# shiinamiyuki/akari_render

Hardware: AMD Instinct MI355X
Metric: Msamples/s (whole node), 1080p path tracer, C2 (higher is better)
Workload: dtype f32

## Files before the change

### akari_render_amd/csrc/device/disect.h

```cpp
#pragma once
#include "drng.h"
#include "dscene.h"
#include "../kernels.h"

namespace akr {

template <bool V>
struct BoolTag {
    static constexpr bool value = V;
};

struct Hit {
    float t, u, v;
    uint32_t gid;
};

struct PlaneHit {
    float t, px, py, pz;
};
AKR_HD PlaneHit tri_plane(vec3 o, vec3 d, float4 r2) {
    float dz = __builtin_fmaf(r2.x, d.x, __builtin_fmaf(r2.y, d.y, r2.z * d.z));
    float oz = __builtin_fmaf(r2.x, o.x, __builtin_fmaf(r2.y, o.y, __builtin_fmaf(r2.z, o.z, r2.w)));
    PlaneHit h;
    h.t = div_f(-oz, dz);
    h.px = __builtin_fmaf(h.t, d.x, o.x);
    h.py = __builtin_fmaf(h.t, d.y, o.y);
    h.pz = __builtin_fmaf(h.t, d.z, o.z);
    return h;
}
AKR_HD void tri_uv(const PlaneHit& h, float4 r0, float4 r1, float& u, float& v) {
    u = __builtin_fmaf(r0.x, h.px, __builtin_fmaf(r0.y, h.py, __builtin_fmaf(r0.z, h.pz, r0.w)));
    v = __builtin_fmaf(r1.x, h.px, __builtin_fmaf(r1.y, h.py, __builtin_fmaf(r1.z, h.pz, r1.w)));
}
AKR_HD bool tri_test(vec3 o, vec3 d, float4 r0, float4 r1, float4 r2, float tmin, float tmax, float& t_out, float& u_out,
                     float& v_out) {
    PlaneHit h = tri_plane(o, d, r2);
    float u, v;
    tri_uv(h, r0, r1, u, v);
    t_out = h.t;
    u_out = u;
    v_out = v;
    return (h.t >= tmin) & (h.t <= tmax) & (u >= 0.0f) & (v >= 0.0f) & (u + v <= 1.0f);
}

AKR_D float textured_alpha(const DScene& sc, const float4* r, uint32_t material, float u, float v) {
    float w = 1.0f - u - v;
    vec2 uv = mk2((r[0].w * w + r[2].w * u) + r[4].w * v, (r[1].w * w + r[3].w * u) + r[5].w * v);
    return material_alpha_at(sc.tex, sc.materials[material], material, uv);
}
template <bool TEX>
AKR_D bool alpha_test(const DScene& sc, uint32_t gid, float u, float v) {
    const float4* r = sc.shade + (size_t)gid * SHADE_ROWS;
    float4 q6 = r[6];
    const DMaterial& m = sc.materials[f2u(q6.y)];
    float alpha = (m.kind == MAT_PRINCIPLED || m.kind == MAT_DIFFUSE) ? m.base_alpha : 1.0f;
    if (TEX) {
        if (m.flags & MF_ALPHA_TEXTURED)
            alpha = textured_alpha(sc, r, f2u(q6.y), u, v);
    }
    if (alpha >= 1.0f) return true;
    uint32_t inst = f2u(q6.z);
    uint32_t prim = gid - sc.inst_tri_offset[inst];
    float h = (float)xxhash32_4(inst, prim, f2u(u), f2u(v)) * 2.3283064365386963e-10f;
    return alpha > h;
}

AKR_D float next_up(float x) {
    uint32_t b = f2u(x);
    return x > 0.0f ? u2f(b + 1u) : (x < 0.0f ? u2f(b - 1u) : u2f(1u));
}
AKR_D float hit_margin(float t, float u, float v, float tmax) {
    return __builtin_fminf(__builtin_fminf(__builtin_fminf(u, v), 1.0f - (u + v)), __builtin_fminf(t, tmax - t));
}

template <bool ANY_HIT, bool TEX = false>
AKR_D bool trace_exhaustive(const DScene& sc, vec3 o, vec3 d, float tmin, float tmax, uint32_t ex0, uint32_t ex1, Hit& hit) {
    float best_t = next_up(tmax);
    uint32_t best = kInvalid;
    float best_u = 0.0f, best_v = 0.0f;
    const uint32_t n = sc.n_tris;
    typedef const float __attribute__((address_space(4))) * ConstF;
    ConstF recs = (ConstF)(uintptr_t)sc.woop;
    auto load_rec = [&](uint32_t k, float4& a, float4& b, float4& c) {
        ConstF r = recs + 12 * (size_t)k;
        a = make_float4(r[0], r[1], r[2], r[3]);
        b = make_float4(r[4], r[5], r[6], r[7]);
        c = make_float4(r[8], r[9], r[10], r[11]);
    };
    float4 n0, n1, n2;
    load_rec(0, n0, n1, n2);
    PlaneHit ph{0.0f, 0.0f, 0.0f, 0.0f};
    for (uint32_t k = 0; k < n; k++) {
        const float4 r0 = n0, r1 = n1, r2 = n2;
        load_rec(k + 1, n0, n1, n2);
        if (!((sc.plane_share_mask >> k) & 1ull)) ph = tri_plane(o, d, r2);
        float u, v;
        const float t = ph.t;
        tri_uv(ph, r0, r1, u, v);
        float m = __builtin_fminf(hit_margin(t, u, v, tmax), t - tmin);
        m = (k == ex0) ? -1.0f : m;
        m = (k == ex1) ? -1.0f : m;
        if (sc.has_alpha) {
            if (m >= 0.0f && !alpha_test<TEX>(sc, k, u, v)) m = -1.0f;
        }
        if (ANY_HIT) {
            if (m >= 0.0f) best = k;
            if (__builtin_amdgcn_ballot_w64(best == kInvalid) == 0) break;
        } else {
            const float tc = (m >= 0.0f) ? t : __builtin_inff();
            const bool better = tc < best_t;
            best_t = better ? tc : best_t;
            best_u = better ? u : best_u;
            best_v = better ? v : best_v;
            best = better ? k : best;
        }
    }
    hit.t = best != kInvalid ? best_t : tmax;
    hit.u = best_u;
    hit.v = best_v;
    hit.gid = best;
    return best != kInvalid;
}

typedef float v2f __attribute__((ext_vector_type(2)));
typedef float v4f __attribute__((ext_vector_type(4)));
AKR_D float min_raw(float a, float b) {
    float r;
    asm("v_min_f32 %0, %1, %2" : "=v"(r) : "v"(a), "v"(b));
    return r;
}
AKR_D float max_raw(float a, float b) {
    float r;
    asm("v_max_f32 %0, %1, %2" : "=v"(r) : "v"(a), "v"(b));
    return r;
}
AKR_D float min_abs_raw(float a, float b) {
    float r;
    asm("v_min_f32 %0, %1, |%2|" : "=v"(r) : "v"(a), "v"(b));
    return r;
}
AKR_D float max3_abs_raw(float a, float b, float c) {
    float r;
    asm("v_max3_f32 %0, |%1|, |%2|, |%3|" : "=v"(r) : "v"(a), "v"(b), "v"(c));
    return r;
}
AKR_D PlaneHit tri_plane_unscaled(vec3 o, vec3 d, float4 r2, float& lo) {
    float dz = __builtin_fmaf(r2.x, d.x, __builtin_fmaf(r2.y, d.y, r2.z * d.z));
    float oz = __builtin_fmaf(r2.x, o.x, __builtin_fmaf(r2.y, o.y, __builtin_fmaf(r2.z, o.z, r2.w)));
    lo = min_abs_raw(lo, oz);
    PlaneHit h;
    h.t = div_f_unscaled(-oz, dz);
    h.px = __builtin_fmaf(h.t, d.x, o.x);
    h.py = __builtin_fmaf(h.t, d.y, o.y);
    h.pz = __builtin_fmaf(h.t, d.z, o.z);
    return h;
}

template <bool DIV>
struct WalkOpt {
    static constexpr bool unscaled_div = DIV;
};
template <int V>
struct IntTag {
    static constexpr int value = V;
};

template <bool TEX = false, class OPT = WalkOpt<true>>
AKR_D void trace_pair_exhaustive(const DScene& sc, vec3 o, vec3 d, float tmax, uint32_t ex0, vec3 so, vec3 sd, float stmax,
                                 uint32_t sex0, uint32_t sex1, Hit& hit, bool& found, bool& occluded, const float4* lds_recs, uint32_t* took_ieee_walk = nullptr) {
    constexpr bool UNSCALED = OPT::unscaled_div && !AKR_RX;
    float best_t = next_up(tmax);
    uint32_t best = kInvalid;
    float best_u = 0.0f, best_v = 0.0f;
    float occ_margin = -1.0f;
    const uint32_t n = sc.n_tris;
    const v4f* lrec = (const v4f*)lds_recs;
    const bool has_alpha = __builtin_amdgcn_readfirstlane((int)sc.has_alpha) != 0;
    float T = 0.0f, srange = 0.0f;
    v2f hx2 = {0.0f, 0.0f}, hy2 = {0.0f, 0.0f}, hz2 = {0.0f, 0.0f};
    float lo = __builtin_inff(), slo = __builtin_inff();
    auto record = [&](auto alpha_tag, auto div_tag, uint32_t k, const v4f& q0, const v4f& q1, const v4f& q2) {
        constexpr int ALPHA = decltype(alpha_tag)::value;
        constexpr bool FAST = decltype(div_tag)::value;
        if (!((sc.plane_share_mask >> k) & 1ull)) {
            const float4 r2 = make_float4(q2.x, q2.y, q2.z, q2.w);
            const PlaneHit a = FAST ? tri_plane_unscaled(o, d, r2, lo) : tri_plane(o, d, r2), b = FAST ? tri_plane_unscaled(so, sd, r2, slo) : tri_plane(so, sd, r2);
            T = a.t;
            srange = min_raw(b.t, stmax - b.t);
            hx2 = (v2f){a.px, b.px}; hy2 = (v2f){a.py, b.py}; hz2 = (v2f){a.pz, b.pz};
        }
        float u, v, su, sv;
        tri_uv(PlaneHit{T, hx2.x, hy2.x, hz2.x}, make_float4(q0.x, q0.y, q0.z, q0.w), make_float4(q1.x, q1.y, q1.z, q1.w), u, v);
        tri_uv(PlaneHit{0.0f, hx2.y, hy2.y, hz2.y}, make_float4(q0.x, q0.y, q0.z, q0.w), make_float4(q1.x, q1.y, q1.z, q1.w), su, sv);
        const v2f u2 = {u, su}, v2 = {v, sv};
        const v2f s2 = {1.0f - (u2.x + v2.x), 1.0f - (u2.y + v2.y)};
        const float range = ALPHA == 0 ? T : min_raw(T, tmax - T);
        float m = min_raw(min_raw(min_raw(u2.x, v2.x), s2.x), range);
        float sm = min_raw(min_raw(min_raw(u2.y, v2.y), s2.y), srange);
        m = (k == ex0) ? -1.0f : m;
        sm = (k == sex0) ? -1.0f : sm;
        sm = (k == sex1) ? -1.0f : sm;
        if (ALPHA == 1 || (ALPHA == 2 && has_alpha)) {
            const uint32_t ka = __builtin_amdgcn_readfirstlane(k);
            if (m >= 0.0f && !alpha_test<TEX>(sc, ka, u2.x, v2.x)) m = -1.0f;
            if (sm >= 0.0f && !alpha_test<TEX>(sc, ka, u2.y, v2.y)) sm = -1.0f;
        }
        const bool better = (m >= 0.0f) & (T < best_t);
        best_t = better ? T : best_t;
        best = better ? k : best;
        occ_margin = max_raw(occ_margin, sm);
    };
    auto walk = [&](auto alpha_tag) {
        const BoolTag<UNSCALED> div_tag{};
        v4f a0 = lrec[0], a1 = lrec[1], a2 = lrec[2], b0, b1, b2;
        uint32_t k = 0;
        for (; k + 1 < n; k += 2) {
            b0 = lrec[3 * (k + 1)]; b1 = lrec[3 * (k + 1) + 1]; b2 = lrec[3 * (k + 1) + 2];
            record(alpha_tag, div_tag, k, a0, a1, a2);
            a0 = lrec[3 * (k + 2)]; a1 = lrec[3 * (k + 2) + 1]; a2 = lrec[3 * (k + 2) + 2];
            record(alpha_tag, div_tag, k + 1, b0, b1, b2);
        }
        if (k < n) record(alpha_tag, div_tag, k, a0, a1, a2);
    };
    auto walk_ieee = [&] {
        best_t = next_up(tmax); best = kInvalid; occ_margin = -1.0f;
#pragma clang loop unroll(disable)
        for (uint32_t k = 0; k < n; k++) {
            record(IntTag<2>{}, BoolTag<false>{}, k, lrec[3 * k], lrec[3 * k + 1], lrec[3 * k + 2]);
        }
    };
    if (UNSCALED) {
        const float ob = lds_recs[3u * (n + 1u) + 2u].w;
        const bool pre_bad = ((tmax >= 0.0f) & !((max3_abs_raw(o.x, o.y, o.z) <= ob) & (max3_abs_raw(d.x, d.y, d.z) <= 2.0f) & (tmax <= 1e20f))) |
                             ((stmax >= 0.0f) & !((max3_abs_raw(so.x, so.y, so.z) <= ob) & (max3_abs_raw(sd.x, sd.y, sd.z) <= 2.0f) & (stmax <= 1e20f)));
        bool redo = __builtin_amdgcn_ballot_w64(pre_bad) != 0;
        if (!redo) {
            if (has_alpha) walk(IntTag<1>{});
            else walk(IntTag<0>{});
            const bool bad = ((tmax >= 0.0f) & (lo < 0x1p-47f)) | ((stmax >= 0.0f) & (slo < 0x1p-47f));
            redo = __builtin_amdgcn_ballot_w64(bad) != 0;
        }
        if (redo) walk_ieee();
        if (took_ieee_walk) *took_ieee_walk = redo ? 1u : 0u;
    } else {
        if (has_alpha) walk(IntTag<1>{});
        else walk(IntTag<0>{});
        if (took_ieee_walk) *took_ieee_walk = 0u;
    }
    if (best != kInvalid) {
        const v4f q0 = lrec[3 * best], q1 = lrec[3 * best + 1];
        const float px = __builtin_fmaf(best_t, d.x, o.x), py = __builtin_fmaf(best_t, d.y, o.y), pz = __builtin_fmaf(best_t, d.z, o.z);
        best_u = __builtin_fmaf(q0.x, px, __builtin_fmaf(q0.y, py, __builtin_fmaf(q0.z, pz, q0.w)));
        best_v = __builtin_fmaf(q1.x, px, __builtin_fmaf(q1.y, py, __builtin_fmaf(q1.z, pz, q1.w)));
    }
    found = best != kInvalid;
    hit.t = found ? best_t : tmax;
    hit.u = best_u;
    hit.v = best_v;
    hit.gid = best;
    occluded = occ_margin >= 0.0f;
}

constexpr uint32_t kBvhDone = 0xfffffffeu;

struct TraceCounters {
    uint32_t nodes, tris, overflow;
};

AKR_D float safe_inv(float d) {
    float a = abs_f(d) < 1e-20f ? __builtin_copysignf(1e-20f, d) : d;
    return __builtin_amdgcn_rcpf(a);
}
AKR_D uint32_t byte_of(uint32_t w, int i) { return (w >> (8 * i)) & 0xffu; }

struct Trav {
    vec3 o, d, inv, noi;
    float tmin, tmax, best_t, best_u, best_v;
    uint32_t ex0, ex1, best;
    uint32_t G, T, tbase, sp, octinv4;
    bool active;
};
AKR_D void trav_begin(Trav& s, vec3 o, vec3 d, float tmin, float tmax, uint32_t ex0, uint32_t ex1) {
    s.o = o; s.d = d;
    s.inv = mk3(safe_inv(d.x), safe_inv(d.y), safe_inv(d.z));
    s.noi = mk3(-o.x * s.inv.x, -o.y * s.inv.y, -o.z * s.inv.z);
    s.tmin = tmin; s.tmax = tmax;
    s.best_t = tmax; s.best_u = 0.0f; s.best_v = 0.0f; s.best = kInvalid;
    s.ex0 = ex0; s.ex1 = ex1;
    const uint32_t oi = (s.inv.x >= 0.0f ? 1u : 0u) | (s.inv.y >= 0.0f ? 2u : 0u) | (s.inv.z >= 0.0f ? 4u : 0u);
    s.octinv4 = oi * 0x01010101u;
    s.G = 1u << (24u + oi);
    s.T = 0; s.tbase = 0; s.sp = 0;
    s.active = tmax >= tmin;
}

AKR_D uint32_t node_pop(Trav& s, uint32_t* __restrict__ stack, uint32_t depth, TraceCounters& cnt) {
    const uint32_t j = 31u - (uint32_t)__builtin_clz(s.G);
    s.G &= ~(1u << j);
    if ((s.G >> 24) != 0) {
        if (s.sp < depth) {
            stack[s.sp * 256u] = s.G;
            s.sp++;
        } else {
            cnt.overflow = 1;
        }
    }
    const uint32_t slot = (j - 24u) ^ (s.octinv4 & 7u);
    return (s.G & 0xffffffu) + slot;
}
AKR_D void hit_commit(Trav& s, bool any_hit, uint32_t gid, float t, float u, float v) {
    if (any_hit) {
        s.best = gid;
        s.T = 0; s.G = 0; s.sp = 0;
    } else {
        const bool better = (s.best == kInvalid) | (t < s.best_t) | ((t == s.best_t) & (gid < s.best));
        if (better) { s.best_t = t; s.best_u = u; s.best_v = v; s.best = gid; }
    }
}
template <bool TEX>
AKR_D void hit_accept(const DScene& sc, Trav& s, bool any_hit, uint32_t gid, float t, float u, float v) {
    bool h = (gid != s.ex0) & (gid != s.ex1);
    if (h && sc.has_alpha) h = alpha_test<TEX>(sc, gid, u, v);
    if (h) hit_commit(s, any_hit, gid, t, u, v);
}

template <int MODE, bool TEX, bool TILE = false>
AKR_D void trav_step_staged(const DScene& sc, Trav& s, uint32_t* __restrict__ stack, TraceCounters& cnt, bool any_rt = false, const uint4* tile = nullptr) {
    const bool any_hit = MODE == 2 ? any_rt : (MODE == 1);
    if (s.T == 0) {
        if ((s.G >> 24) == 0) {
            s.sp--;
            s.G = stack[s.sp * 256u];
        }
        const uint32_t idx = node_pop(s, stack, sc.bvh_stack_depth, cnt);
        const uint4* p = sc.bvh_nodes + (size_t)idx * (kBvhNodeWords / 4);
        uint4 w0, w1, w2, w3;
        if (TILE && idx < sc.bvh_tile_nodes) {
            typedef const volatile uint32_t __attribute__((address_space(3))) * LdsW;
            typedef uint32_t u32x4 __attribute__((ext_vector_type(4)));
            typedef const volatile u32x4 __attribute__((address_space(3))) * LdsU4;
            LdsU4 pt = (LdsU4)((LdsW)(const uint32_t*)tile + idx * kBvhNodeWords);
            const u32x4 t0 = pt[0], t1 = pt[1], t2 = pt[2], t3 = pt[3];
            w0 = make_uint4(t0.x, t0.y, t0.z, t0.w); w1 = make_uint4(t1.x, t1.y, t1.z, t1.w); w2 = make_uint4(t2.x, t2.y, t2.z, t2.w);
            w3 = make_uint4(t3.x, t3.y, t3.z, t3.w);
        } else {
            w0 = p[0]; w1 = p[1]; w2 = p[2]; w3 = p[3];
        }
        cnt.nodes++;
        const float limit = s.best_t;
        const float bx = u2f((w0.w & 0xffu) << 23) * s.inv.x, by = u2f(((w0.w >> 8) & 0xffu) << 23) * s.inv.y, bz = u2f(((w0.w >> 16) & 0xffu) << 23) * s.inv.z;
        const float ax = __builtin_fmaf(u2f(w0.x), s.inv.x, s.noi.x), ay = __builtin_fmaf(u2f(w0.y), s.inv.y, s.noi.y), az = __builtin_fmaf(u2f(w0.z), s.inv.z, s.noi.z);
        const bool nx = s.inv.x < 0.0f, ny = s.inv.y < 0.0f, nz = s.inv.z < 0.0f;
        const uint32_t xb = nx ? ((w3.y >> 16) | (w3.y << 16)) : w3.y, yb = ny ? ((w3.z >> 16) | (w3.z << 16)) : w3.z, zb = nz ? ((w3.w >> 16) | (w3.w << 16)) : w3.w;
        const uint32_t qnx[2] = {nx ? w2.z : w1.w, xb}, qfx[2] = {nx ? w1.w : w2.z, xb >> 16};
        const uint32_t qny[2] = {ny ? w2.w : w2.x, yb}, qfy[2] = {ny ? w2.x : w2.w, yb >> 16};
        const uint32_t qnz[2] = {nz ? w3.x : w2.y, zb}, qfz[2] = {nz ? w2.y : w3.x, zb >> 16};
        uint32_t hitmask = 0;
#pragma unroll
        for (int h = 0; h < 2; h++) {
            const uint32_t meta4 = h ? (w1.x >> 16) : w1.y;
            const uint32_t is_inner4 = (meta4 & (meta4 << 1)) & 0x10101010u;
            const uint32_t inner_mask4 = (is_inner4 >> 4) * 0xffu;
            const uint32_t bit_index4 = (meta4 ^ (s.octinv4 & inner_mask4)) & 0x1f1f1f1fu;
            const uint32_t child_bits4 = (meta4 >> 5) & 0x07070707u;
#pragma unroll
            for (int i = 0; i < (h ? 2 : 4); i++) {
                const float tnx = __builtin_fmaf((float)byte_of(qnx[h], i), bx, ax), tfx = __builtin_fmaf((float)byte_of(qfx[h], i), bx, ax);
                const float tny = __builtin_fmaf((float)byte_of(qny[h], i), by, ay), tfy = __builtin_fmaf((float)byte_of(qfy[h], i), by, ay);
                const float tnz = __builtin_fmaf((float)byte_of(qnz[h], i), bz, az), tfz = __builtin_fmaf((float)byte_of(qfz[h], i), bz, az);
                const float tn = __builtin_fmaxf(__builtin_fmaxf(tnx, tny), __builtin_fmaxf(tnz, s.tmin));
                const float tf = __builtin_fminf(__builtin_fminf(tfx, tfy), __builtin_fminf(tfz, limit));
                if (tn <= tf) hitmask |= byte_of(child_bits4, i) << byte_of(bit_index4, i);
            }
        }
        s.G = ((w0.w >> 24) | ((w1.x & 0xffffu) << 8)) | (hitmask & 0xff000000u);
        s.T = hitmask & 0x00ffffffu;
        s.tbase = w1.z;
    }
    if (s.T != 0) {
        const uint32_t b = (uint32_t)__builtin_ctz(s.T);
        s.T &= s.T - 1u;
        const uint4* p = (const uint4*)sc.woop + (size_t)(s.tbase + b) * (kBvhTriWords / 4);
        const uint4 w0 = p[0], w1 = p[1], w2 = p[2], w3 = p[3];
        cnt.tris++;
        float t, u, v;
        bool h = tri_test(s.o, s.d, make_float4(u2f(w0.x), u2f(w0.y), u2f(w0.z), u2f(w0.w)), make_float4(u2f(w1.x), u2f(w1.y), u2f(w1.z), u2f(w1.w)),
                          make_float4(u2f(w2.x), u2f(w2.y), u2f(w2.z), u2f(w2.w)), s.tmin, s.tmax, t, u, v);
        if (h) hit_accept<TEX>(sc, s, any_hit, w3.x, t, u, v);
    }
    s.active = (s.T != 0) | ((s.G >> 24) != 0) | (s.sp != 0);
}
template <int MODE, bool TEX, bool TILE = false>
AKR_D void trav_step(const DScene& sc, Trav& s, uint32_t* __restrict__ stack, TraceCounters& cnt, bool any_rt = false, const uint4* tile = nullptr) {
    if constexpr (TEX) {
        trav_step_staged<MODE, TEX, TILE>(sc, s, stack, cnt, any_rt, tile);
        return;
    }
    const bool any_hit = MODE == 2 ? any_rt : (MODE == 1);
    const bool do_tri = s.T != 0;
    const uint4* p;
    bool in_tile = false;
    uint32_t tile_idx = 0;
    if (do_tri) {
        const uint32_t b = (uint32_t)__builtin_ctz(s.T);
        s.T &= s.T - 1u;
        p = (const uint4*)sc.woop + (size_t)(s.tbase + b) * (kBvhTriWords / 4);
    } else {
        if ((s.G >> 24) == 0) {
            s.sp--;
            s.G = stack[s.sp * 256u];
        }
        const uint32_t idx = node_pop(s, stack, sc.bvh_stack_depth, cnt);
        p = sc.bvh_nodes + (size_t)idx * (kBvhNodeWords / 4);
        if (TILE && idx < sc.bvh_tile_nodes) {
            in_tile = true;
            tile_idx = idx;
        }
    }
    uint4 w0, w1, w2, w3;
    if (TILE && in_tile) {
        typedef const volatile uint32_t __attribute__((address_space(3))) * LdsW;
        typedef uint32_t u32x4 __attribute__((ext_vector_type(4)));
        typedef const volatile u32x4 __attribute__((address_space(3))) * LdsU4;
        LdsU4 pt = (LdsU4)((LdsW)(const uint32_t*)tile + tile_idx * kBvhNodeWords);
        const u32x4 t0 = pt[0], t1 = pt[1], t2 = pt[2], t3 = pt[3];
        w0 = make_uint4(t0.x, t0.y, t0.z, t0.w); w1 = make_uint4(t1.x, t1.y, t1.z, t1.w); w2 = make_uint4(t2.x, t2.y, t2.z, t2.w);
        w3 = make_uint4(t3.x, t3.y, t3.z, t3.w);
    } else {
        w0 = p[0]; w1 = p[1]; w2 = p[2]; w3 = p[3];
    }
    asm volatile("" : "+v"(w0.x), "+v"(w0.y), "+v"(w0.z), "+v"(w0.w), "+v"(w1.x), "+v"(w1.y), "+v"(w1.z), "+v"(w1.w), "+v"(w2.x), "+v"(w2.y),
                      "+v"(w2.z), "+v"(w2.w), "+v"(w3.x), "+v"(w3.y), "+v"(w3.z), "+v"(w3.w));
    if (do_tri) {
        cnt.tris++;
        float t, u, v;
        bool h = tri_test(s.o, s.d, make_float4(u2f(w0.x), u2f(w0.y), u2f(w0.z), u2f(w0.w)), make_float4(u2f(w1.x), u2f(w1.y), u2f(w1.z), u2f(w1.w)),
                          make_float4(u2f(w2.x), u2f(w2.y), u2f(w2.z), u2f(w2.w)), s.tmin, s.tmax, t, u, v);
        if (h) {
            const uint32_t gid = w3.x;
            h = (gid != s.ex0) & (gid != s.ex1);
            if (h && sc.has_alpha) h = alpha_test<TEX>(sc, gid, u, v);
            if (h) {
                if (any_hit) {
                    s.best = gid;
                    s.T = 0; s.G = 0; s.sp = 0;
                } else {
                    const bool better = (s.best == kInvalid) | (t < s.best_t) | ((t == s.best_t) & (gid < s.best));
                    if (better) { s.best_t = t; s.best_u = u; s.best_v = v; s.best = gid; }
                }
            }
        }
    } else {
        cnt.nodes++;
        const float limit = s.best_t;
        const float bx = u2f((w0.w & 0xffu) << 23) * s.inv.x, by = u2f(((w0.w >> 8) & 0xffu) << 23) * s.inv.y, bz = u2f(((w0.w >> 16) & 0xffu) << 23) * s.inv.z;
        const float ax = __builtin_fmaf(u2f(w0.x), s.inv.x, s.noi.x), ay = __builtin_fmaf(u2f(w0.y), s.inv.y, s.noi.y), az = __builtin_fmaf(u2f(w0.z), s.inv.z, s.noi.z);
        const bool nx = s.inv.x < 0.0f, ny = s.inv.y < 0.0f, nz = s.inv.z < 0.0f;
        const uint32_t xb = nx ? ((w3.y >> 16) | (w3.y << 16)) : w3.y, yb = ny ? ((w3.z >> 16) | (w3.z << 16)) : w3.z, zb = nz ? ((w3.w >> 16) | (w3.w << 16)) : w3.w;
        const uint32_t qnx[2] = {nx ? w2.z : w1.w, xb}, qfx[2] = {nx ? w1.w : w2.z, xb >> 16};
        const uint32_t qny[2] = {ny ? w2.w : w2.x, yb}, qfy[2] = {ny ? w2.x : w2.w, yb >> 16};
        const uint32_t qnz[2] = {nz ? w3.x : w2.y, zb}, qfz[2] = {nz ? w2.y : w3.x, zb >> 16};
        uint32_t hitmask = 0;
#pragma unroll
        for (int h = 0; h < 2; h++) {
            const uint32_t meta4 = h ? (w1.x >> 16) : w1.y;
            const uint32_t is_inner4 = (meta4 & (meta4 << 1)) & 0x10101010u;
            const uint32_t inner_mask4 = (is_inner4 >> 4) * 0xffu;
            const uint32_t bit_index4 = (meta4 ^ (s.octinv4 & inner_mask4)) & 0x1f1f1f1fu;
            const uint32_t child_bits4 = (meta4 >> 5) & 0x07070707u;
#pragma unroll
            for (int i = 0; i < (h ? 2 : 4); i++) {
                const float tnx = __builtin_fmaf((float)byte_of(qnx[h], i), bx, ax), tfx = __builtin_fmaf((float)byte_of(qfx[h], i), bx, ax);
                const float tny = __builtin_fmaf((float)byte_of(qny[h], i), by, ay), tfy = __builtin_fmaf((float)byte_of(qfy[h], i), by, ay);
                const float tnz = __builtin_fmaf((float)byte_of(qnz[h], i), bz, az), tfz = __builtin_fmaf((float)byte_of(qfz[h], i), bz, az);
                const float tn = __builtin_fmaxf(__builtin_fmaxf(tnx, tny), __builtin_fmaxf(tnz, s.tmin));
                const float tf = __builtin_fminf(__builtin_fminf(tfx, tfy), __builtin_fminf(tfz, limit));
                if (tn <= tf) hitmask |= byte_of(child_bits4, i) << byte_of(bit_index4, i);
            }
        }
        s.G = ((w0.w >> 24) | ((w1.x & 0xffffu) << 8)) | (hitmask & 0xff000000u);
        s.T = hitmask & 0x00ffffffu;
        s.tbase = w1.z;
    }
    s.active = (s.T != 0) | ((s.G >> 24) != 0) | (s.sp != 0);
}

template <bool ANY_HIT, bool TEX = false>
AKR_D bool trace_bvh(const DScene& sc, vec3 o, vec3 d, float tmin, float tmax, uint32_t ex0, uint32_t ex1, Hit& hit,
                     uint32_t* __restrict__ stack, TraceCounters& cnt) {
    Trav s;
    trav_begin(s, o, d, tmin, tmax, ex0, ex1);
    while (s.active) trav_step<ANY_HIT ? 1 : 0, TEX>(sc, s, stack, cnt);
    hit.t = s.best_t; hit.u = s.best_u; hit.v = s.best_v; hit.gid = s.best;
    return s.best != kInvalid;
}

AKR_D uint4 carry_best(const Trav& s) { return make_uint4(f2u(s.best_t), f2u(s.best_u), f2u(s.best_v), s.best); }
AKR_D uint4 carry_place(const Trav& s) { return make_uint4(s.G, s.T, s.tbase, s.sp); }
AKR_D void trav_resume(const DScene& sc, Trav& s, uint4 best, uint4 place) {
    s.best_t = u2f(best.x); s.best_u = u2f(best.y); s.best_v = u2f(best.z); s.best = best.w;
    s.G = place.x; s.T = place.y; s.tbase = place.z; s.sp = place.w;
    s.active = (s.T != 0) | ((s.G >> 24) != 0) | (s.sp != 0);
}

}
```

Measured before the change: 3793.

## Merge plane-sharing triangle pairs in exhaustive walk using wave-wide lane masks

Splits the per-triangle record into plane solve and barycentric margin steps. In the non-alpha walk it processes triangle pairs with ballot/inverse-ballot lane masks. When two triangles share a plane, the t<best_t comparison and best update are done once for the pair, and exclusion checks are precomputed as pair-level masks. The aim is fewer per-triangle compares and selects in the hot loop, at the cost of scalar mask bookkeeping and more intricate tie-ordering logic.

```diff
diff --git a/akari_render_amd/csrc/device/disect.h b/akari_render_amd/csrc/device/disect.h
--- a/akari_render_amd/csrc/device/disect.h
+++ b/akari_render_amd/csrc/device/disect.h
@@ -144,6 +144,8 @@
     asm("v_max3_f32 %0, |%1|, |%2|, |%3|" : "=v"(r) : "v"(a), "v"(b), "v"(c));
     return r;
 }
+AKR_D uint64_t lanes_of(bool c) { return __builtin_amdgcn_ballot_w64(c); }
+AKR_D bool in_lanes(uint64_t m) { return __builtin_amdgcn_inverse_ballot_w64(m); }
 AKR_D PlaneHit tri_plane_unscaled(vec3 o, vec3 d, float4 r2, float& lo) {
     float dz = __builtin_fmaf(r2.x, d.x, __builtin_fmaf(r2.y, d.y, r2.z * d.z));
     float oz = __builtin_fmaf(r2.x, o.x, __builtin_fmaf(r2.y, o.y, __builtin_fmaf(r2.z, o.z, r2.w)));
@@ -156,9 +158,17 @@
     return h;
 }
 
-template <bool DIV>
+#ifndef AKR_WALK_PLANE_LT
+#define AKR_WALK_PLANE_LT 1
+#endif
+#ifndef AKR_WALK_PLANE_EXCL
+#define AKR_WALK_PLANE_EXCL 1
+#endif
+template <bool DIV, bool LT = DIV && AKR_WALK_PLANE_LT, bool EXCL = DIV && AKR_WALK_PLANE_EXCL>
 struct WalkOpt {
     static constexpr bool unscaled_div = DIV;
+    static constexpr bool plane_lt = LT;
+    static constexpr bool plane_excl = EXCL;
 };
 template <int V>
 struct IntTag {
@@ -179,24 +189,31 @@
     float T = 0.0f, srange = 0.0f;
     v2f hx2 = {0.0f, 0.0f}, hy2 = {0.0f, 0.0f}, hz2 = {0.0f, 0.0f};
     float lo = __builtin_inff(), slo = __builtin_inff();
-    auto record = [&](auto alpha_tag, auto div_tag, uint32_t k, const v4f& q0, const v4f& q1, const v4f& q2) {
+    auto solve = [&](auto div_tag, const v4f& q2) {
+        constexpr bool FAST = decltype(div_tag)::value;
+        const float4 r2 = make_float4(q2.x, q2.y, q2.z, q2.w);
+        const PlaneHit a = FAST ? tri_plane_unscaled(o, d, r2, lo) : tri_plane(o, d, r2), b = FAST ? tri_plane_unscaled(so, sd, r2, slo) : tri_plane(so, sd, r2);
+        T = a.t;
+        srange = min_raw(b.t, stmax - b.t);
+        hx2 = (v2f){a.px, b.px}; hy2 = (v2f){a.py, b.py}; hz2 = (v2f){a.pz, b.pz};
+    };
+    auto margins = [&](auto alpha_tag, const v4f& q0, const v4f& q1, v2f& u2, v2f& v2, float& m, float& sm) {
         constexpr int ALPHA = decltype(alpha_tag)::value;
-        constexpr bool FAST = decltype(div_tag)::value;
-        if (!((sc.plane_share_mask >> k) & 1ull)) {
-            const float4 r2 = make_float4(q2.x, q2.y, q2.z, q2.w);
-            const PlaneHit a = FAST ? tri_plane_unscaled(o, d, r2, lo) : tri_plane(o, d, r2), b = FAST ? tri_plane_unscaled(so, sd, r2, slo) : tri_plane(so, sd, r2);
-            T = a.t;
-            srange = min_raw(b.t, stmax - b.t);
-            hx2 = (v2f){a.px, b.px}; hy2 = (v2f){a.py, b.py}; hz2 = (v2f){a.pz, b.pz};
-        }
         float u, v, su, sv;
         tri_uv(PlaneHit{T, hx2.x, hy2.x, hz2.x}, make_float4(q0.x, q0.y, q0.z, q0.w), make_float4(q1.x, q1.y, q1.z, q1.w), u, v);
         tri_uv(PlaneHit{0.0f, hx2.y, hy2.y, hz2.y}, make_float4(q0.x, q0.y, q0.z, q0.w), make_float4(q1.x, q1.y, q1.z, q1.w), su, sv);
-        const v2f u2 = {u, su}, v2 = {v, sv};
+        u2 = (v2f){u, su}; v2 = (v2f){v, sv};
         const v2f s2 = {1.0f - (u2.x + v2.x), 1.0f - (u2.y + v2.y)};
         const float range = ALPHA == 0 ? T : min_raw(T, tmax - T);
-        float m = min_raw(min_raw(min_raw(u2.x, v2.x), s2.x), range);
-        float sm = min_raw(min_raw(min_raw(u2.y, v2.y), s2.y), srange);
+        m = min_raw(min_raw(min_raw(u2.x, v2.x), s2.x), range);
+        sm = min_raw(min_raw(min_raw(u2.y, v2.y), s2.y), srange);
+    };
+    auto record = [&](auto alpha_tag, auto div_tag, uint32_t k, const v4f& q0, const v4f& q1, const v4f& q2) {
+        constexpr int ALPHA = decltype(alpha_tag)::value;
+        if (!((sc.plane_share_mask >> k) & 1ull)) solve(div_tag, q2);
+        v2f u2, v2;
+        float m, sm;
+        margins(alpha_tag, q0, q1, u2, v2, m, sm);
         m = (k == ex0) ? -1.0f : m;
         sm = (k == sex0) ? -1.0f : sm;
         sm = (k == sex1) ? -1.0f : sm;
@@ -212,13 +229,65 @@
     };
     auto walk = [&](auto alpha_tag) {
         const BoolTag<UNSCALED> div_tag{};
+        constexpr bool PLANE_LT = OPT::plane_lt && decltype(alpha_tag)::value == 0, PLANE_EXCL = OPT::plane_excl && decltype(alpha_tag)::value == 0;
         v4f a0 = lrec[0], a1 = lrec[1], a2 = lrec[2], b0, b1, b2;
         uint32_t k = 0;
-        for (; k + 1 < n; k += 2) {
-            b0 = lrec[3 * (k + 1)]; b1 = lrec[3 * (k + 1) + 1]; b2 = lrec[3 * (k + 1) + 2];
-            record(alpha_tag, div_tag, k, a0, a1, a2);
-            a0 = lrec[3 * (k + 2)]; a1 = lrec[3 * (k + 2) + 1]; a2 = lrec[3 * (k + 2) + 2];
-            record(alpha_tag, div_tag, k + 1, b0, b1, b2);
+        if (PLANE_LT || PLANE_EXCL) {
+            const uint32_t qex0 = ex0 | 1u, qsex0 = sex0 | 1u, qsex1 = sex1 | 1u;
+            const uint64_t hex0 = lanes_of((ex0 & 1u) != 0), hsex0 = lanes_of((sex0 & 1u) != 0), hsex1 = lanes_of((sex1 & 1u) != 0);
+            auto choose = [&](uint64_t acc, uint32_t id) {
+                const uint64_t better = acc & lanes_of(T < best_t);
+                best_t = in_lanes(better) ? T : best_t;
+                best = in_lanes(better) ? id : best;
+            };
+            for (; k + 1 < n; k += 2) {
+                b0 = lrec[3 * (k + 1)]; b1 = lrec[3 * (k + 1) + 1]; b2 = lrec[3 * (k + 1) + 2];
+                const uint32_t k1 = k + 1;
+                const bool own_b = !((sc.plane_share_mask >> k1) & 1ull);
+                uint64_t xa, xb, sxa, sxb;
+                if (PLANE_EXCL) {
+                    const uint64_t e = lanes_of(qex0 == k1), s0 = lanes_of(qsex0 == k1), s1 = lanes_of(qsex1 == k1);
+                    xa = e & ~hex0; xb = e & hex0;
+                    sxa = (s0 & ~hsex0) | (s1 & ~hsex1); sxb = (s0 & hsex0) | (s1 & hsex1);
+                } else {
+                    xa = lanes_of(k == ex0); xb = lanes_of(k1 == ex0);
+                    sxa = lanes_of(k == sex0) | lanes_of(k == sex1); sxb = lanes_of(k1 == sex0) | lanes_of(k1 == sex1);
+                }
+                v2f u2, v2;
+                float ma, sma, mb, smb;
+                if (!((sc.plane_share_mask >> k) & 1ull)) solve(div_tag, a2);
+                margins(alpha_tag, a0, a1, u2, v2, ma, sma);
+                sma = in_lanes(sxa) ? -1.0f : sma;
+                uint64_t acc_a = lanes_of(ma >= 0.0f) & ~xa;
+                a0 = lrec[3 * (k + 2)]; a1 = lrec[3 * (k + 2) + 1]; a2 = lrec[3 * (k + 2) + 2];
+                if (!PLANE_LT) choose(acc_a, k);
+                if (own_b) {
+                    if (PLANE_LT) {
+                        choose(acc_a, k);
+                        acc_a = 0;
+                    }
+                    solve(div_tag, b2);
+                }
+                margins(alpha_tag, b0, b1, u2, v2, mb, smb);
+                smb = in_lanes(sxb) ? -1.0f : smb;
+                const uint64_t acc_b = lanes_of(mb >= 0.0f) & ~xb;
+                if (PLANE_LT) {
+                    const uint64_t lt = lanes_of(T < best_t);
+                    best_t = in_lanes((acc_a | acc_b) & lt) ? T : best_t;
+                    best = in_lanes(acc_b & lt) ? k1 : best;
+                    best = in_lanes(acc_a & lt) ? k : best;
+                } else {
+                    choose(acc_b, k1);
+                }
+                occ_margin = max_raw(max_raw(occ_margin, sma), smb);
+            }
+        } else {
+            for (; k + 1 < n; k += 2) {
+                b0 = lrec[3 * (k + 1)]; b1 = lrec[3 * (k + 1) + 1]; b2 = lrec[3 * (k + 1) + 2];
+                record(alpha_tag, div_tag, k, a0, a1, a2);
+                a0 = lrec[3 * (k + 2)]; a1 = lrec[3 * (k + 2) + 1]; a2 = lrec[3 * (k + 2) + 2];
+                record(alpha_tag, div_tag, k + 1, b0, b1, b2);
+            }
         }
         if (k < n) record(alpha_tag, div_tag, k, a0, a1, a2);
     };
```

Measured after the change: 3839 (median of 6 runs). 1.01x the previous value.
